# krea-ai/realtime-video

Measured on AMD Instinct MI355X. Metric: frames/sec at 832x480, 4-step 14B T2V (per-step DiT latency in config), higher is better.
Workload: dtype bf16

## Files before the change

### realtime_video_amd/csrc/gemm8.hip

```cpp
#include <atomic>
#include <mutex>
#include <type_traits>

#include "gemm_core.h"
#include "gemm_split.h"
#include "rtv_internal.h"

namespace rtv {

namespace g8 {
constexpr int BM = 256, BN = 256, BK = 64;
constexpr int HALF_BYTES = 128 * BK * 2;
constexpr int A_OFF = 0;
constexpr int W_OFF = 6 * HALF_BYTES;
constexpr int LDS_BYTES = 10 * HALF_BYTES;
constexpr int THREADS = 512;
__device__ __forceinline__ int swz(int row, int chunk) { return chunk ^ ((row >> 1) & 7); }
}

#ifdef RTV_GEMM_TIMELINE
__device__ unsigned long long* g_timeline = nullptr;
#endif

__device__ __forceinline__ void g8_tile_mn(int tiles_m, int tiles_n, int tile_id, int* mt, int* nt) {
#if RTV_G8_BALANCED_GROUPS
  const int ngrp = (tiles_m + 7) >> 3;
  const int gq = tiles_m / ngrp, gr = tiles_m - gq * ngrp;
  const int big = (gq + 1) * tiles_n;
  int first_m, gm, in_group;
  if (tile_id < gr * big) {
    const int group = tile_id / big;
    gm = gq + 1;
    first_m = group * gm;
    in_group = tile_id - group * big;
  } else {
    const int t = tile_id - gr * big, sm = gq * tiles_n, group = t / sm;
    gm = gq;
    first_m = gr * (gq + 1) + group * gq;
    in_group = t - group * sm;
  }
#else
  constexpr int GROUP_M = 8;
  const int per_group = GROUP_M * tiles_n;
  const int group = tile_id / per_group;
  const int first_m = group * GROUP_M;
  const int gm = min(tiles_m - first_m, GROUP_M);
  const int in_group = tile_id - group * per_group;
#endif
  *mt = first_m + in_group % gm;
  *nt = in_group / gm;
}

template <bool F16>
__device__ __forceinline__ void gemm8m_body(const GemmParams& p, const SplitArgs& sp, int m0, int n0, int tile_id, int seg, int unit,
                                            int kt_begin, int kt_end, bool is_split);

template <bool F16, bool SKIP_IDLE>
__global__ __launch_bounds__(g8::THREADS, 2) void gemm8_kernel(GemmParams p, SplitArgs sp) {
  using namespace g8;
  int bid0 = blockIdx.x;
  if (sp.pair_units) {
    if (bid0 < sp.pair_pad) {
      if (bid0 >= sp.pair_units) return;
#pragma unroll 1
      for (int j = 0; j < 2; ++j) {
        const int tn = 2 * bid0 + j;
        if (tn >= p.tiles_n) break;
        if (j) __syncthreads();
        gemm8m_body<F16>(p, sp, sp.pair_m0, tn * BN, 0, 0, -1, 0, p.K / BK, false);
      }
      return;
    }
    bid0 -= sp.pair_pad;
  }
  if (sp.half_tail) {
    const int nhu = 2 * sp.tail_tiles;
    if (sp.split_first) bid0 = bid0 < nhu ? sp.first_unit + bid0 : bid0 - nhu;
    if (bid0 >= sp.first_unit) {
      const int v = xcd_remap(bid0 - sp.first_unit, nhu);
      const int tile_id = sp.first_unit + (v >> 1);
      int mt, nt;
      g8_tile_mn(p.tiles_m, p.tiles_n, tile_id, &mt, &nt);
      const int m0h = mt * BM + (v & 1) * 128;
      if (m0h >= p.M) return;
      gemm8m_body<F16>(p, sp, m0h, nt * BN, tile_id, 0, -1, 0, p.K / BK, false);
      return;
    }
    sp.S = 1;
    sp.split_first = 0;
  }
#ifdef RTV_GEMM_TIMELINE
  const unsigned long long tl_t0 = __builtin_amdgcn_s_memrealtime();
  unsigned long long tl_t1 = 0;
#endif
  typedef TileCfg<256, 256, 64, 2, 4> Cfg;
  extern __shared__ __attribute__((aligned(16))) char smem[];

  const int tid = threadIdx.x;
  const int lane = tid & 63;
  const int wave = __builtin_amdgcn_readfirstlane(tid >> 6);
  const int wr = wave >> 2, wc = wave & 3;
  const int l31 = lane & 31, g = lane >> 5;

  const int nk_total = p.K / BK;
  int tile_id, seg, unit, kt_begin, kt_end;
  const bool is_split = split_unit_of_block(sp, bid0, nk_total, &tile_id, &unit, &seg, &kt_begin, &kt_end);
  int mt_, nt_;
  g8_tile_mn(p.tiles_m, p.tiles_n, tile_id, &mt_, &nt_);
  const int m0 = mt_ * BM;
  const int n0 = nt_ * BN;
  uint32_t src_off[4][2];
  {
    const int rsub = lane >> 3, cpos = lane & 7;
#pragma unroll
    for (int j = 0; j < 2; ++j) {
      const int row = j * 64 + wave * 8 + rsub;
      const int ch = swz(row, cpos) * 8;
#pragma unroll
      for (int h = 0; h < 2; ++h) {
        const int gm_row = min(m0 + h * 128 + row, p.M - 1);
        const int gn_row = min(n0 + h * 128 + row, p.N - 1);
        src_off[h][j] = ((uint32_t)gm_row * (uint32_t)p.lda + ch) * 2u;
        src_off[2 + h][j] = ((uint32_t)gn_row * (uint32_t)p.ldw + ch) * 2u;
      }
    }
  }
  __amdgpu_buffer_rsrc_t rsrcA = __builtin_amdgcn_make_buffer_rsrc((void*)p.A, 0, 0x7fffffff, 0x00020000);
  __amdgpu_buffer_rsrc_t rsrcW = __builtin_amdgcn_make_buffer_rsrc((void*)p.W, 0, 0x7fffffff, 0x00020000);
  auto stage_piece = [&](int kt, int a3, int h, int j, auto chk) {
    if (decltype(chk)::value && kt >= kt_end) return;
    const int slot = h < 2 ? A_OFF + (a3 * 2 + h) * HALF_BYTES : W_OFF + ((kt & 1) * 2 + (h - 2)) * HALF_BYTES;
    __builtin_amdgcn_raw_ptr_buffer_load_lds(h < 2 ? rsrcA : rsrcW, (RTV_LDS void*)(smem + slot + (j * 64 + wave * 8) * 128), 16,
                                             src_off[h][j], (unsigned)kt * (BK * 2), 0, 0);
  };

  const int b_row0 = (wc & 1) * 64;
  u32x4 af[2][4];
  u32x4 bfr[2][4];
  auto read_a = [&](int a3, int mq) {
    const char* s = smem + A_OFF + (a3 * 2 + wr) * HALF_BYTES;
#pragma unroll
    for (int mb = 0; mb < 2; ++mb) {
      const int row = mq * 64 + mb * 32 + l31;
#pragma unroll
      for (int ks = 0; ks < 4; ++ks) af[mb][ks] = *(const u32x4*)(s + row * 128 + (swz(row, ks * 2 + g) << 4));
    }
  };
  auto read_w = [&](int wb) {
    const char* s = smem + W_OFF + (wb * 2 + (wc >> 1)) * HALF_BYTES;
#pragma unroll
    for (int nq = 0; nq < 2; ++nq) {
      const int row = b_row0 + nq * 32 + l31;
#pragma unroll
      for (int ks = 0; ks < 4; ++ks) bfr[nq][ks] = *(const u32x4*)(s + row * 128 + (swz(row, ks * 2 + g) << 4));
    }
  };

  f32x16 acc[4][2];
#pragma unroll
  for (int mi = 0; mi < 4; ++mi)
#pragma unroll
    for (int ni = 0; ni < 2; ++ni)
#pragma unroll
      for (int r = 0; r < 16; ++r) acc[mi][ni][r] = 0.f;

#define G8_FENCE() __builtin_amdgcn_sched_barrier(0)
#define G8_BARRIER()                  \
  do {                                \
    G8_FENCE();                       \
    __builtin_amdgcn_s_barrier();     \
    G8_FENCE();                       \
  } while (0)
#define G8_LDS_DONE()                                   \
  do {                                                  \
    asm volatile("s_waitcnt lgkmcnt(0)" ::: "memory");  \
    G8_FENCE();                                         \
  } while (0)

  const bool idle_rows = SKIP_IDLE && m0 + wr * 128 >= p.M;
  auto mma_half = [&](int mq, int st_kt, int st_a3, int h0, auto chk) {
    __builtin_amdgcn_s_setprio(1);
    int n = 0;
#pragma unroll
    for (int ks = 0; ks < 4; ++ks)
#pragma unroll
      for (int nq = 0; nq < 2; ++nq)
#pragma unroll
        for (int mb = 0; mb < 2; ++mb) {
          acc[mq * 2 + mb][nq] = Mfma32<F16>::run(bfr[nq][ks], af[mb][ks], acc[mq * 2 + mb][nq]);
          ++n;
          if ((n & 3) == 2) {
            G8_FENCE();
            stage_piece(st_kt, st_a3, h0 + (n >> 3), (n >> 2) & 1, chk);
            G8_FENCE();
          }
        }
    __builtin_amdgcn_s_setprio(0);
  };

#pragma unroll
  for (int t = 0; t < 2; ++t)
#pragma unroll
    for (int hh = 0; hh < 4; ++hh) {
      const int h = (hh + 2) & 3;
      stage_piece(kt_begin + t, t, h, 0, std::true_type{});
      stage_piece(kt_begin + t, t, h, 1, std::true_type{});
    }
  if (kt_begin + 1 < kt_end) asm volatile("s_waitcnt vmcnt(8)" ::: "memory");
  else asm volatile("s_waitcnt vmcnt(0)" ::: "memory");
  G8_BARRIER();
  if (wr == 1) G8_BARRIER();

  int a3 = 0;
  auto k_tile = [&](const int kt, auto chk) {
    constexpr bool CHK = decltype(chk)::value;
    const int a3n = a3 == 0 ? 2 : a3 - 1;
    read_w(kt & 1);
    read_a(a3, 0);
    G8_LDS_DONE();
    G8_BARRIER();
    mma_half(0, kt + 2, a3n, 0, chk);
    G8_BARRIER();
    read_a(a3, 1);
    if (!CHK || kt + 2 < kt_end) asm volatile("s_waitcnt vmcnt(4)" ::: "memory");
    else asm volatile("s_waitcnt vmcnt(0)" ::: "memory");
    G8_LDS_DONE();
    G8_BARRIER();
    mma_half(1, kt + 2, a3n, 2, chk);
    G8_BARRIER();
    a3 = a3 == 2 ? 0 : a3 + 1;
  };
  auto idle_tile = [&](const int kt) {
    const int a3n = a3 == 0 ? 2 : a3 - 1;
    G8_BARRIER();
#pragma unroll
    for (int i = 0; i < 4; ++i) stage_piece(kt + 2, a3n, i >> 1, i & 1, std::true_type{});
    G8_BARRIER();
    if (kt + 2 < kt_end) asm volatile("s_waitcnt vmcnt(4)" ::: "memory");
    else asm volatile("s_waitcnt vmcnt(0)" ::: "memory");
    G8_BARRIER();
#pragma unroll
    for (int i = 0; i < 4; ++i) stage_piece(kt + 2, a3n, 2 + (i >> 1), i & 1, std::true_type{});
    G8_BARRIER();
    a3 = a3 == 2 ? 0 : a3 + 1;
  };
  int kt = kt_begin;
  if (idle_rows) {
    for (; kt < kt_end; ++kt) idle_tile(kt);
  } else {
    for (; kt + 2 < kt_end; ++kt) k_tile(kt, std::false_type{});
    for (; kt < kt_end; ++kt) k_tile(kt, std::true_type{});
  }
  if (wr == 0) G8_BARRIER();

#ifdef RTV_GEMM_TIMELINE
  tl_t1 = __builtin_amdgcn_s_memrealtime();
  bool reducer = true;
  if (is_split) reducer = split_k_reduce<4>(acc, sp, unit, seg, tile_id, smem, tid, wave, lane);
  if (!reducer) {
    if (g_timeline && tid == 0) {
      unsigned long long* t = g_timeline + (size_t)blockIdx.x * 4;
      t[0] = tl_t0;
      t[1] = tl_t1;
      t[2] = __builtin_amdgcn_s_memrealtime();
      t[3] = ((unsigned long long)(seg + 1) << 32) | (unsigned)tile_id;
    }
    return;
  }
#else
  if (is_split && !split_k_reduce<4>(acc, sp, unit, seg, tile_id, smem, tid, wave, lane)) return;
#endif

  const bool wide = !((p.ldc | (p.residual ? p.ldr : 0)) & 7) && !(((uintptr_t)p.C | (uintptr_t)p.residual) & 15);
  if (wide) {
    if (is_split) __syncthreads();
#ifdef RTV_GEMM_TIMELINE
    unsigned long long tl_mid = 0;
    store_tile_lds<F16, 4>(p, m0 + wr * 128, n0 + wc * 64, lane, smem + wave * (128 * 128), acc, &tl_mid);
    if (g_timeline && tid == 0) g_timeline[(size_t)blockIdx.x * 4 + 1] = tl_mid | (1ull << 63);
    tl_t1 = tl_t1 ? tl_t1 : 0;
    if (g_timeline && tid == 0) {
      unsigned long long* t = g_timeline + (size_t)blockIdx.x * 4;
      t[0] = tl_t0;
      t[2] = __builtin_amdgcn_s_memrealtime();
      t[3] = ((unsigned long long)(is_split ? seg + 1 : 0) << 32) | (unsigned)tile_id;
      g_timeline[(size_t)(gridDim.x + blockIdx.x) * 4] = tl_t1;
    }
    return;
#else
    store_tile_lds<F16, 4>(p, m0 + wr * 128, n0 + wc * 64, lane, smem + wave * (128 * 128), acc);
#endif
  } else {
    store_tile<F16, Cfg>(p, m0 + wr * 128, n0 + wc * 64, lane, acc);
  }
#ifdef RTV_GEMM_TIMELINE
  if (g_timeline && tid == 0) {
    unsigned long long* t = g_timeline + (size_t)blockIdx.x * 4;
    t[0] = tl_t0;
    t[1] = tl_t1;
    t[2] = __builtin_amdgcn_s_memrealtime();
    t[3] = ((unsigned long long)(is_split ? seg + 1 : 0) << 32) | (unsigned)tile_id | (is_split ? 0x80000000u : 0u);
  }
#endif
}

static std::atomic<bool> g_gemm8_skip_idle{true};
static std::atomic<bool> g_gemm8_half_tail{true};
static std::atomic<bool> g_gemm8_ragged_strips{true};
namespace g8m {
constexpr int BM = 128, BN = 256, BK = 64;
constexpr int HALF_BYTES = 128 * BK * 2;
constexpr int LDS_BYTES = 9 * HALF_BYTES;
}

template <bool F16>
__device__ __forceinline__ void gemm8m_body(const GemmParams& p, const SplitArgs& sp, int m0, int n0, int tile_id, int seg, int unit,
                                            int kt_begin, int kt_end, bool is_split) {
  using namespace g8m;
  extern __shared__ __attribute__((aligned(16))) char smem[];
  const int tid = threadIdx.x;
  const int lane = tid & 63;
  const int wave = __builtin_amdgcn_readfirstlane(tid >> 6);
  const int wr = wave >> 2, wc = wave & 3;
  const int l31 = lane & 31, g = lane >> 5;

  uint32_t src_off[3][2];
  {
    const int rsub = lane >> 3, cpos = lane & 7;
#pragma unroll
    for (int j = 0; j < 2; ++j) {
      const int row = j * 64 + wave * 8 + rsub;
      const int ch = g8::swz(row, cpos) * 8;
      src_off[0][j] = ((uint32_t)min(m0 + row, p.M - 1) * (uint32_t)p.lda + ch) * 2u;
      src_off[1][j] = ((uint32_t)min(n0 + row, p.N - 1) * (uint32_t)p.ldw + ch) * 2u;
      src_off[2][j] = ((uint32_t)min(n0 + 128 + row, p.N - 1) * (uint32_t)p.ldw + ch) * 2u;
    }
  }
  __amdgpu_buffer_rsrc_t rsrcA = __builtin_amdgcn_make_buffer_rsrc((void*)p.A, 0, 0x7fffffff, 0x00020000);
  __amdgpu_buffer_rsrc_t rsrcW = __builtin_amdgcn_make_buffer_rsrc((void*)p.W, 0, 0x7fffffff, 0x00020000);
  auto stage_piece = [&](int kt, int b3, int h, int j, auto chk) {
    if (decltype(chk)::value && kt >= kt_end) return;
    __builtin_amdgcn_raw_ptr_buffer_load_lds(h == 0 ? rsrcA : rsrcW,
                                             (RTV_LDS void*)(smem + (b3 * 3 + h) * HALF_BYTES + (j * 64 + wave * 8) * 128), 16,
                                             src_off[h][j], (unsigned)kt * (BK * 2), 0, 0);
  };

  u32x4 af[2][4], bfr[2][4];
  auto read_frags = [&](int b3) {
    const char* sa = smem + (b3 * 3) * HALF_BYTES;
    const char* sw = smem + (b3 * 3 + 1 + (wc >> 1)) * HALF_BYTES;
#pragma unroll
    for (int nq = 0; nq < 2; ++nq) {
      const int row = (wc & 1) * 64 + nq * 32 + l31;
#pragma unroll
      for (int ks = 0; ks < 4; ++ks) bfr[nq][ks] = *(const u32x4*)(sw + row * 128 + (g8::swz(row, ks * 2 + g) << 4));
    }
#pragma unroll
    for (int mb = 0; mb < 2; ++mb) {
      const int row = wr * 64 + mb * 32 + l31;
#pragma unroll
      for (int ks = 0; ks < 4; ++ks) af[mb][ks] = *(const u32x4*)(sa + row * 128 + (g8::swz(row, ks * 2 + g) << 4));
    }
  };

  f32x16 acc[2][2];
#pragma unroll
  for (int mi = 0; mi < 2; ++mi)
#pragma unroll
    for (int ni = 0; ni < 2; ++ni)
#pragma unroll
      for (int r = 0; r < 16; ++r) acc[mi][ni][r] = 0.f;

#pragma unroll
  for (int t = 0; t < 2; ++t)
#pragma unroll
    for (int h = 0; h < 3; ++h) {
      stage_piece(kt_begin + t, t, h, 0, std::true_type{});
      stage_piece(kt_begin + t, t, h, 1, std::true_type{});
    }
  if (wr == 1) {
#pragma unroll
    for (int h = 0; h < 3; ++h) {
      stage_piece(kt_begin + 2, 2, h, 0, std::true_type{});
      stage_piece(kt_begin + 2, 2, h, 1, std::true_type{});
    }
  }
  if (wr == 1) {
    if (kt_begin + 2 < kt_end) asm volatile("s_waitcnt vmcnt(6)" ::: "memory");
    else asm volatile("s_waitcnt vmcnt(0)" ::: "memory");
  } else {
    if (kt_begin + 1 < kt_end) asm volatile("s_waitcnt vmcnt(6)" ::: "memory");
    else asm volatile("s_waitcnt vmcnt(0)" ::: "memory");
  }
  G8_BARRIER();
  if (wr == 1) G8_BARRIER();

  int b3 = 0;
  auto k_tile = [&](const int kt, auto chk) {
    constexpr bool CHK = decltype(chk)::value;
    read_frags(b3);
    G8_LDS_DONE();
    G8_BARRIER();
    const int st_kt = kt + 2 + wr;
    const int st_b = wr ? b3 : (b3 == 0 ? 2 : b3 - 1);
    __builtin_amdgcn_s_setprio(1);
    int n = 0;
#pragma unroll
    for (int ks = 0; ks < 4; ++ks)
#pragma unroll
      for (int nq = 0; nq < 2; ++nq)
#pragma unroll
        for (int mb = 0; mb < 2; ++mb) {
          acc[mb][nq] = Mfma32<F16>::run(bfr[nq][ks], af[mb][ks], acc[mb][nq]);
          ++n;
          if (n == 2 || n == 4 || n == 7 || n == 10 || n == 12 || n == 15) {
            const int pc = n == 2 ? 0 : n == 4 ? 1 : n == 7 ? 2 : n == 10 ? 3 : n == 12 ? 4 : 5;
            G8_FENCE();
            stage_piece(st_kt, st_b, pc >> 1, pc & 1, chk);
            G8_FENCE();
          }
        }
    __builtin_amdgcn_s_setprio(0);
    G8_FENCE();
    if (!CHK || st_kt < kt_end) asm volatile("s_waitcnt vmcnt(6)" ::: "memory");
    else asm volatile("s_waitcnt vmcnt(0)" ::: "memory");
    G8_BARRIER();
    b3 = b3 == 2 ? 0 : b3 + 1;
  };
  int kt = kt_begin;
  for (; kt + 3 < kt_end; ++kt) k_tile(kt, std::false_type{});
  for (; kt < kt_end; ++kt) k_tile(kt, std::true_type{});
  if (wr == 0) G8_BARRIER();

  if (is_split && !split_k_reduce<2>(acc, sp, unit, seg, tile_id, smem, tid, wave, lane)) return;

  const bool wide = !((p.ldc | (p.residual ? p.ldr : 0)) & 7) && !(((uintptr_t)p.C | (uintptr_t)p.residual) & 15);
  if (wide) {
    if (is_split) __syncthreads();
    store_tile_lds<F16, 2>(p, m0 + wr * 64, n0 + wc * 64, lane, smem + wave * (64 * 128), acc);
  } else {
    typedef TileCfg<128, 256, 64, 2, 4> CfgM;
    store_tile<F16, CfgM>(p, m0 + wr * 64, n0 + wc * 64, lane, acc);
  }
}

template <bool F16>
__global__ __launch_bounds__(g8::THREADS, 2) void gemm8m_kernel(GemmParams p, SplitArgs sp) {
  using namespace g8m;
  const int nk_total = p.K / BK;
  int tile_id, seg, unit, kt_begin, kt_end;
  const bool is_split = split_unit_of_block(sp, blockIdx.x, nk_total, &tile_id, &unit, &seg, &kt_begin, &kt_end);
  constexpr int GROUP_M = 8;
  const int per_group = GROUP_M * p.tiles_n;
  const int group = tile_id / per_group;
  const int first_m = group * GROUP_M;
  const int gm = min(p.tiles_m - first_m, GROUP_M);
  const int in_group = tile_id - group * per_group;
  gemm8m_body<F16>(p, sp, (first_m + in_group % gm) * BM, (in_group / gm) * BN, tile_id, seg, unit, kt_begin, kt_end, is_split);
}

struct SplitWorkspace {
  int device;
  hipStream_t stream;
  bool any_stream;
  float* slabs;
  int* counters;
};
constexpr int MAX_WORKSPACES = 64;
constexpr int MAX_DEVICES = 64;
static SplitWorkspace g_ws[MAX_WORKSPACES];
static int g_num_ws = 0;
static std::mutex g_ws_mu;

static int attach_workspace(bool any_stream, hipStream_t stream, void* ptr, size_t bytes) {
  int dev = 0;
  if (hipGetDevice(&dev) != hipSuccess) return set_error(-1, "gemm_set_workspace: cannot query the device");
  std::lock_guard<std::mutex> lk(g_ws_mu);
  int slot = -1;
  for (int i = 0; i < g_num_ws; ++i)
    if (g_ws[i].device == dev && g_ws[i].any_stream == any_stream && (any_stream || g_ws[i].stream == stream)) slot = i;
  if (!ptr) {
    if (slot >= 0) g_ws[slot] = g_ws[--g_num_ws];
    return 0;
  }
  if (((uintptr_t)ptr) & 255) return set_error(-1, "gemm_set_workspace: pointer must be 256-byte aligned");
  if (bytes < rtv_gemm_workspace_bytes()) return set_error(-1, "gemm_set_workspace: too small (rtv_gemm_workspace_bytes)");
  if (slot < 0) {
    if (g_num_ws == MAX_WORKSPACES) return set_error(-1, "gemm_set_workspace: too many workspaces attached");
    slot = g_num_ws++;
  }
  SplitWorkspace w{dev, stream, any_stream, (float*)ptr, (int*)((char*)ptr + (size_t)SPLIT_MAX_UNITS * SPLIT_SLAB_FLOATS * 4)};
  if (hipMemset(w.counters, 0, (size_t)SPLIT_MAX_UNITS * sizeof(int)) != hipSuccess) {
    if (slot == g_num_ws - 1) --g_num_ws;
    return set_error(-1, "gemm_set_workspace: cannot zero the arrival counters");
  }
  g_ws[slot] = w;
  return 0;
}

}

using namespace rtv;

#ifdef RTV_GEMM_TIMELINE
extern "C" int rtv_gemm_debug_timeline(unsigned long long* buf) {
  return hipMemcpyToSymbol(HIP_SYMBOL(g_timeline), &buf, sizeof(buf)) == hipSuccess ? 0 : -1;
}
#endif

extern "C" int rtv_gemm_set_half_tail(int on) {
  rtv::g_gemm8_half_tail.store(on != 0, std::memory_order_relaxed);
  return 0;
}

extern "C" int rtv_gemm_set_ragged_strips(int on) {
  rtv::g_gemm8_ragged_strips.store(on != 0, std::memory_order_relaxed);
  return 0;
}

extern "C" int rtv_gemm_set_skip_idle(int on) {
  rtv::g_gemm8_skip_idle.store(on != 0, std::memory_order_relaxed);
  return 0;
}

extern "C" size_t rtv_gemm_workspace_bytes(void) {
  return (size_t)SPLIT_MAX_UNITS * SPLIT_SLAB_FLOATS * 4 + (size_t)SPLIT_MAX_UNITS * 4 + 256;
}

extern "C" int rtv_gemm_set_workspace(void* ptr, size_t bytes) { return attach_workspace(true, nullptr, ptr, bytes); }

extern "C" int rtv_gemm_set_stream_workspace(rtv_stream_t stream, void* ptr, size_t bytes) {
  return attach_workspace(false, (hipStream_t)stream, ptr, bytes);
}

namespace rtv {

int plan_split_k(int T, int nk, bool allow_split, SplitArgs* sp, int* grid, hipStream_t stream, bool allow_half, int extra_units) {
  int dev = 0;
  if (hipGetDevice(&dev) != hipSuccess || dev < 0 || dev >= MAX_DEVICES) return set_error(-1, "gemm: cannot query the device");
  float* slabs = nullptr;
  int* counters = nullptr;
  const int G = device_num_cus();
  if (G <= 0) return set_error(-1, "gemm: cannot query the device");
  {
    std::lock_guard<std::mutex> lk(g_ws_mu);
    for (int i = 0; i < g_num_ws && allow_split; ++i) {
      const SplitWorkspace& w = g_ws[i];
      if (w.device != dev) continue;
      if (!w.any_stream && w.stream == stream) {
        slabs = w.slabs;
        counters = w.counters;
        break;
      }
      if (w.any_stream && !slabs) {
        slabs = w.slabs;
        counters = w.counters;
      }
    }
  }
  *sp = SplitArgs{T, 1, nullptr, nullptr, 0, 0, 0, 0, 0, 0};
  *grid = T;
  const int R = (T + extra_units) % G <= T ? (T + extra_units) % G : 0;
  if (allow_half && g_gemm8_half_tail.load(std::memory_order_relaxed) && R > 0 && T > R && G / R == 2 && nk <= 128) {
    sp->first_unit = T - R;
    sp->tail_tiles = R;
    sp->half_tail = 1;
    *grid = (T - R) + 2 * R;
    return 0;
  }
  if (allow_split && slabs && R > 0) {
    int S = G / R;
    if (S > 8) S = 8;
    if (S > nk / 4) S = nk / 4;
    if (S >= 2 && (size_t)R * S <= (size_t)SPLIT_MAX_UNITS) {
      sp->first_unit = T - R;
      sp->S = S;
      sp->slabs = slabs;
      sp->counters = counters;
      sp->tail_tiles = R;
      sp->split_first = (R * S * 4 <= G) ? 1 : 0;
      *grid = (T - R) + R * S;
    }
  }
  return 0;
}

template <bool F16, bool SKIP_IDLE>
static int launch_gemm8_t(GemmParams p, bool allow_split, hipStream_t stream) {
  p.tiles_m = (p.M + g8::BM - 1) / g8::BM;
  p.tiles_n = (p.N + g8::BN - 1) / g8::BN;
  auto kern = gemm8_kernel<F16, SKIP_IDLE>;
  static LdsAttr lds_attr;
  if (int st = ensure_dynamic_lds((const void*)kern, g8::LDS_BYTES, &lds_attr, "gemm8")) return st;
  SplitArgs sp;
  int grid = 0;
// ... 59 lines not shown
```

### realtime_video_amd/csrc/gemm_core.h

```cpp
#pragma once
#include "rtv_common.h"

namespace rtv {

struct GemmParams {
  const uint16_t* A;
  const uint16_t* W;
  uint16_t* C;
  int lda, ldw, ldc;
  int M, N, K;
  const uint16_t* bias;
  int act;
  const uint16_t* gate;
  int gate_stride;
  int rows_per_frame;
  int row_offset;
  const uint16_t* residual;
  int ldr;
  int tiles_m, tiles_n;
};

template <bool F16>
struct Mfma32;
template <>
struct Mfma32<false> {
  static __device__ __forceinline__ f32x16 run(const u32x4& a, const u32x4& b, const f32x16& c) {
    return __builtin_amdgcn_mfma_f32_32x32x16_bf16(__builtin_bit_cast(bf16x8, a),
                                                   __builtin_bit_cast(bf16x8, b), c, 0, 0, 0);
  }
  static __device__ __forceinline__ float to_f32(uint16_t v) { return bf16_to_f32(v); }
  static __device__ __forceinline__ uint16_t from_f32(float v) { return f32_to_bf16(v); }
  static __device__ __forceinline__ float round(float v) { return round_bf16(v); }
  static __device__ __forceinline__ uint32_t pack2(float lo, float hi) { return pack_bf16x2(lo, hi); }
  static __device__ __forceinline__ float lo_f32(uint32_t u) { return __uint_as_float(u << 16); }
  static __device__ __forceinline__ float hi_f32(uint32_t u) { return __uint_as_float(u & 0xffff0000u); }
};
template <>
struct Mfma32<true> {
  static __device__ __forceinline__ f32x16 run(const u32x4& a, const u32x4& b, const f32x16& c) {
    return __builtin_amdgcn_mfma_f32_32x32x16_f16(__builtin_bit_cast(f16x8, a),
                                                  __builtin_bit_cast(f16x8, b), c, 0, 0, 0);
  }
  static __device__ __forceinline__ float to_f32(uint16_t v) { return f16_to_f32(v); }
  static __device__ __forceinline__ uint16_t from_f32(float v) { return f32_to_f16(v); }
  static __device__ __forceinline__ float round(float v) { return round_f16(v); }
  static __device__ __forceinline__ uint32_t pack2(float lo, float hi) { return pack_f16x2(lo, hi); }
  static __device__ __forceinline__ float lo_f32(uint32_t u) { return f16_to_f32((uint16_t)(u & 0xffff)); }
  static __device__ __forceinline__ float hi_f32(uint32_t u) { return f16_to_f32((uint16_t)(u >> 16)); }
};

template <int BM, int BN, int BK, int WM, int WN>
struct TileCfg {
  static constexpr int NW = WM * WN;
  static constexpr int NT = NW * 64;
  static constexpr int CH = BK / 8;
  static constexpr int RPI = 64 / CH;
  static constexpr int RPB = 16 / CH;
  static constexpr int A_INST = BM / RPI / NW;
  static constexpr int B_INST = BN / RPI / NW;
  static constexpr int A_BYTES = BM * BK * 2;
  static constexpr int B_BYTES = BN * BK * 2;
  static constexpr int STAGE_BYTES = A_BYTES + B_BYTES;
  static constexpr int TM = BM / WM / 32;
  static constexpr int TN = BN / WN / 32;
  static_assert(BM % (RPI * NW) == 0 && BN % (RPI * NW) == 0, "tile/wave mismatch");
  static_assert(BK % 16 == 0 && (CH == 4 || CH == 8), "BK must be 32 or 64");
  static __device__ __forceinline__ int swz(int row, int chunk) {
    return chunk ^ ((row / RPB) & (CH - 1));
  }
};

__device__ __forceinline__ void dma16(const void* gsrc, char* lds_wave_base) {
  __builtin_amdgcn_global_load_lds((const RTV_GLOBAL void*)gsrc, (RTV_LDS void*)lds_wave_base, 16, 0,
                                   0);
}

template <bool F16, typename Cfg, int BK>
__device__ __forceinline__ void mma_stage(const char* sA, const char* sB, int a_row0, int b_row0,
                                          int lane, f32x16 (&acc)[Cfg::TM][Cfg::TN]) {
  const int l31 = lane & 31, g = lane >> 5;
#pragma unroll
  for (int ks = 0; ks < BK / 16; ++ks) {
    u32x4 af[Cfg::TM], bf[Cfg::TN];
#pragma unroll
    for (int mi = 0; mi < Cfg::TM; ++mi) {
      int row = a_row0 + mi * 32 + l31;
      af[mi] = *(const u32x4*)(sA + row * (BK * 2) + Cfg::swz(row, ks * 2 + g) * 16);
    }
#pragma unroll
    for (int ni = 0; ni < Cfg::TN; ++ni) {
      int row = b_row0 + ni * 32 + l31;
      bf[ni] = *(const u32x4*)(sB + row * (BK * 2) + Cfg::swz(row, ks * 2 + g) * 16);
    }
#pragma unroll
    for (int mi = 0; mi < Cfg::TM; ++mi)
#pragma unroll
      for (int ni = 0; ni < Cfg::TN; ++ni)
        acc[mi][ni] = Mfma32<F16>::run(bf[ni], af[mi], acc[mi][ni]);
  }
}

template <bool F16>
__device__ __forceinline__ void epilogue_quad(const GemmParams& p, int m, int n, const float* v4) {
  typedef Mfma32<F16> T;
  float v[4] = {v4[0], v4[1], v4[2], v4[3]};
  if (p.bias) {
    u32x2 b = *(const u32x2*)(p.bias + n);
    v[0] += T::to_f32(b[0] & 0xffff);
    v[1] += T::to_f32(b[0] >> 16);
    v[2] += T::to_f32(b[1] & 0xffff);
    v[3] += T::to_f32(b[1] >> 16);
  }
#pragma unroll
  for (int i = 0; i < 4; ++i) v[i] = T::round(v[i]);
  if (p.act == 1) {
#pragma unroll
    for (int i = 0; i < 4; ++i) v[i] = T::round(gelu_tanh(v[i]));
  } else if (p.act == 2) {
#pragma unroll
    for (int i = 0; i < 4; ++i) v[i] = T::round(silu(v[i]));
  }
  if (p.gate) {
    const uint16_t* gp = p.gate + (size_t)((p.row_offset + m) / p.rows_per_frame) * p.gate_stride + n;
    u32x2 g = *(const u32x2*)gp;
    v[0] = T::round(v[0] * T::to_f32(g[0] & 0xffff));
    v[1] = T::round(v[1] * T::to_f32(g[0] >> 16));
    v[2] = T::round(v[2] * T::to_f32(g[1] & 0xffff));
    v[3] = T::round(v[3] * T::to_f32(g[1] >> 16));
  }
  if (p.residual) {
    u32x2 r = *(const u32x2*)(p.residual + (size_t)m * p.ldr + n);
    v[0] += T::to_f32(r[0] & 0xffff);
    v[1] += T::to_f32(r[0] >> 16);
    v[2] += T::to_f32(r[1] & 0xffff);
    v[3] += T::to_f32(r[1] >> 16);
  }
  u32x2 o;
  o[0] = (uint32_t)T::from_f32(v[0]) | ((uint32_t)T::from_f32(v[1]) << 16);
  o[1] = (uint32_t)T::from_f32(v[2]) | ((uint32_t)T::from_f32(v[3]) << 16);
  *(u32x2*)(p.C + (size_t)m * p.ldc + n) = o;
}

template <bool F16, typename Cfg>
__device__ __forceinline__ void store_tile(const GemmParams& p, int m_base, int n_base, int lane,
                                           f32x16 (&acc)[Cfg::TM][Cfg::TN]) {
  const int l31 = lane & 31, g = lane >> 5;
#pragma unroll
  for (int mi = 0; mi < Cfg::TM; ++mi) {
    int m = m_base + mi * 32 + l31;
    if (m >= p.M) continue;
#pragma unroll
    for (int ni = 0; ni < Cfg::TN; ++ni) {
#pragma unroll
      for (int rq = 0; rq < 4; ++rq) {
        int n = n_base + ni * 32 + rq * 8 + g * 4;
        if (n < p.N) {
          float v4[4] = {acc[mi][ni][rq * 4 + 0], acc[mi][ni][rq * 4 + 1], acc[mi][ni][rq * 4 + 2],
                         acc[mi][ni][rq * 4 + 3]};
          epilogue_quad<F16>(p, m, n, v4);
        }
      }
    }
  }
}

template <bool F16, int TM, int ACT, bool GATE>
__device__ __forceinline__ void store_tile_lds_impl(const GemmParams& p, int m_base, int n_base, int lane, char* img,
                                                    f32x16 (&acc)[TM][2], unsigned long long* mid_stamp) {
  typedef Mfma32<F16> T;
  const int l31 = lane & 31, g = lane >> 5;
  int ncol[8];
  u32x2 bq[8];
#pragma unroll
  for (int s8 = 0; s8 < 8; ++s8) {
    ncol[s8] = min(n_base + (s8 >> 2) * 32 + (s8 & 3) * 8 + g * 4, p.N - 4);
    bq[s8] = p.bias ? *(const u32x2*)(p.bias + ncol[s8]) : u32x2{0u, 0u};
  }
#pragma unroll
  for (int mi = 0; mi < TM; ++mi) {
    const int row = mi * 32 + l31;
    u32x2 gq[8];
    if (GATE) {
      const uint16_t* gp = p.gate + (size_t)((p.row_offset + min(m_base + row, p.M - 1)) / p.rows_per_frame) * p.gate_stride;
#pragma unroll
      for (int s8 = 0; s8 < 8; ++s8) gq[s8] = *(const u32x2*)(gp + ncol[s8]);
    }
#pragma unroll
    for (int ni = 0; ni < 2; ++ni)
#pragma unroll
      for (int rq = 0; rq < 4; ++rq) {
        const int s8 = ni * 4 + rq;
        float v[4] = {acc[mi][ni][rq * 4 + 0], acc[mi][ni][rq * 4 + 1], acc[mi][ni][rq * 4 + 2], acc[mi][ni][rq * 4 + 3]};
        v[0] += T::lo_f32(bq[s8][0]);
        v[1] += T::hi_f32(bq[s8][0]);
        v[2] += T::lo_f32(bq[s8][1]);
        v[3] += T::hi_f32(bq[s8][1]);
        if (ACT == 1) {
#pragma unroll
          for (int i = 0; i < 4; ++i) v[i] = gelu_tanh(T::round(v[i]));
        } else if (ACT == 2) {
#pragma unroll
          for (int i = 0; i < 4; ++i) v[i] = silu(T::round(v[i]));
        }
        if (GATE) {
          v[0] = T::round(v[0]) * T::lo_f32(gq[s8][0]);
          v[1] = T::round(v[1]) * T::hi_f32(gq[s8][0]);
          v[2] = T::round(v[2]) * T::lo_f32(gq[s8][1]);
          v[3] = T::round(v[3]) * T::hi_f32(gq[s8][1]);
        }
        u32x2 o;
        o[0] = T::pack2(v[0], v[1]);
        o[1] = T::pack2(v[2], v[3]);
        const int chunk = s8 ^ (row & 7);
        const int half = g ^ ((row >> 3) & 1);
        *(u32x2*)(img + row * 128 + chunk * 16 + half * 8) = o;
      }
  }
  asm volatile("s_waitcnt lgkmcnt(0)" ::: "memory");
  __builtin_amdgcn_sched_barrier(0);
  if (mid_stamp) *mid_stamp = __builtin_amdgcn_s_memrealtime();
  const int rsub = lane >> 3, c = lane & 7;
  const int n = n_base + c * 8;
  const bool n_ok = n < p.N;
  constexpr int PASSES = TM * 4;
  u32x4 res[PASSES];
  if (p.residual) {
#pragma unroll
    for (int ps = 0; ps < PASSES; ++ps) {
      const int m = min(m_base + ps * 8 + rsub, p.M - 1);
      res[ps] = *(const u32x4*)(p.residual + (size_t)m * p.ldr + min(n, p.N - 8));
    }
  }
#pragma unroll
  for (int ps = 0; ps < PASSES; ++ps) {
    const int row = ps * 8 + rsub;
    const int m = m_base + row;
    u32x4 t = *(const u32x4*)(img + row * 128 + ((c ^ (row & 7)) << 4));
    if ((row >> 3) & 1) t = u32x4{t[2], t[3], t[0], t[1]};
    if (p.residual) {
#pragma unroll
      for (int i = 0; i < 4; ++i)
        t[i] = T::pack2(T::lo_f32(t[i]) + T::lo_f32(res[ps][i]), T::hi_f32(t[i]) + T::hi_f32(res[ps][i]));
    }
    if (m < p.M && n_ok) *(u32x4*)(p.C + (size_t)m * p.ldc + n) = t;
  }
}

template <bool F16, int TM>
__device__ __forceinline__ void store_tile_lds(const GemmParams& p, int m_base, int n_base, int lane, char* img,
                                               f32x16 (&acc)[TM][2], unsigned long long* mid_stamp = nullptr) {
  if (p.gate) {
    if (p.act == 0) store_tile_lds_impl<F16, TM, 0, true>(p, m_base, n_base, lane, img, acc, mid_stamp);
    else if (p.act == 1) store_tile_lds_impl<F16, TM, 1, true>(p, m_base, n_base, lane, img, acc, mid_stamp);
    else store_tile_lds_impl<F16, TM, 2, true>(p, m_base, n_base, lane, img, acc, mid_stamp);
  } else {
    if (p.act == 0) store_tile_lds_impl<F16, TM, 0, false>(p, m_base, n_base, lane, img, acc, mid_stamp);
    else if (p.act == 1) store_tile_lds_impl<F16, TM, 1, false>(p, m_base, n_base, lane, img, acc, mid_stamp);
    else store_tile_lds_impl<F16, TM, 2, false>(p, m_base, n_base, lane, img, acc, mid_stamp);
  }
}

}
```

### realtime_video_amd/csrc/gemm_split.h

```cpp
#pragma once
#include "rtv_common.h"

namespace rtv {

constexpr int SPLIT_SLAB_FLOATS = 256 * 256;
constexpr int SPLIT_MAX_UNITS = 256;

struct SplitArgs {
  int first_unit;
  int S;
  float* slabs;
  int* counters;
  int tail_tiles;
  int split_first;
  int half_tail;
  int pair_units;
  int pair_pad;
  int pair_m0;
};

int plan_split_k(int T, int nk, bool allow_split, SplitArgs* sp, int* grid, hipStream_t stream, bool allow_half = false,
                 int extra_units = 0);

__device__ __forceinline__ bool split_unit_of_block(const SplitArgs& sp, int bid, int nk_total, int* tile_id, int* unit,
                                                    int* seg, int* kt_begin, int* kt_end) {
  *seg = 0;
  *unit = -1;
  if (sp.split_first) {
    const int nsu = sp.tail_tiles * sp.S;
    bid = bid < nsu ? sp.first_unit + bid : bid - nsu;
  }
  if (bid < sp.first_unit) {
    *tile_id = xcd_remap(bid, sp.first_unit);
  } else {
    const int v = xcd_remap(bid - sp.first_unit, sp.tail_tiles * sp.S);
    *seg = v / sp.tail_tiles;
    const int tl = v - *seg * sp.tail_tiles;
    *tile_id = sp.first_unit + tl;
    *unit = tl * sp.S + *seg;
  }
  const bool is_split = *unit >= 0 && sp.S > 1;
  *kt_begin = is_split ? (int)((long)nk_total * *seg / sp.S) : 0;
  *kt_end = is_split ? (int)((long)nk_total * (*seg + 1) / sp.S) : nk_total;
  return is_split;
}

template <int TM>
__device__ __forceinline__ bool split_k_reduce(f32x16 (&acc)[TM][2], const SplitArgs& sp, int unit, int seg, int tile_id,
                                               char* smem, int tid, int wave, int lane) {
  constexpr int NB = TM * 2;
  __amdgpu_buffer_rsrc_t slab =
      __builtin_amdgcn_make_buffer_rsrc((void*)(sp.slabs + (size_t)unit * SPLIT_SLAB_FLOATS), 0, SPLIT_SLAB_FLOATS * 4, 0x00020000);
#pragma unroll
  for (int blk = 0; blk < NB; ++blk)
#pragma unroll
    for (int q = 0; q < 4; ++q) {
      const f32x16& a = acc[blk >> 1][blk & 1];
      const f32x4 v = {a[4 * q], a[4 * q + 1], a[4 * q + 2], a[4 * q + 3]};
      __builtin_amdgcn_raw_buffer_store_b128(__builtin_bit_cast(u32x4, v), slab, (((wave * NB + blk) * 4 + q) * 64 + lane) * 16, 0,
                                              16);
    }
  asm volatile("s_waitcnt vmcnt(0)" ::: "memory");
  __syncthreads();
  int* flag = (int*)smem;
  if (tid == 0)
    *flag = __hip_atomic_fetch_add(sp.counters + (tile_id - sp.first_unit), 1, __ATOMIC_RELAXED, __HIP_MEMORY_SCOPE_AGENT);
  __syncthreads();
  const int ticket = *flag;
  if (ticket != sp.S - 1) return false;
  if (tid == 0) {
    __builtin_amdgcn_fence(__ATOMIC_ACQUIRE, "agent");
    __hip_atomic_store(sp.counters + (tile_id - sp.first_unit), 0, __ATOMIC_RELAXED, __HIP_MEMORY_SCOPE_AGENT);
  }
  __syncthreads();
  const int unit0 = unit - seg;
  if (sp.S > 2) {
#pragma unroll
    for (int blk = 0; blk < NB; ++blk)
#pragma unroll
      for (int r = 0; r < 16; ++r) acc[blk >> 1][blk & 1][r] = 0.f;
  }
  for (int s = 0; s < sp.S; ++s) {
    if (s == seg && sp.S == 2) continue;
    const float4* other = (const float4*)(sp.slabs + (size_t)(unit0 + s) * SPLIT_SLAB_FLOATS);
#pragma unroll
    for (int blk = 0; blk < NB; ++blk)
#pragma unroll
      for (int q = 0; q < 4; ++q) {
        const float4 v = other[((wave * NB + blk) * 4 + q) * 64 + lane];
        f32x16& a = acc[blk >> 1][blk & 1];
        a[4 * q] += v.x;
        a[4 * q + 1] += v.y;
        a[4 * q + 2] += v.z;
        a[4 * q + 3] += v.w;
      }
  }
  return true;
}

}
```

Before: 18.56.

## Switch gemm8 kernels from 32x32x16 to 16x16x32 MFMA with matching epilogues

Replaces the 32x32 MFMA instruction in both gemm8 kernels with the 16x16x32 variant, reorganizing fragment loads, accumulator layout, the interleaving of global-to-LDS staging with MFMAs, the split-K reduction and the tile store epilogues to fit the new 16x16 accumulator shape. It is enabled by default through a compile macro. The intent is higher MFMA throughput or better latency behavior on MI355X for these shapes. It adds more, smaller instructions and LDS reads, and changes register pressure and how staging overlaps with compute.

After: 18.85 (median of 6 runs). +1.6%, better.

```diff
diff --git a/realtime_video_amd/csrc/gemm8.hip b/realtime_video_amd/csrc/gemm8.hip
--- a/realtime_video_amd/csrc/gemm8.hip
+++ b/realtime_video_amd/csrc/gemm8.hip
@@ -5,6 +5,10 @@
 #include "gemm_core.h"
 #include "gemm_split.h"
 #include "rtv_internal.h"
+
+#ifndef RTV_G8_MFMA16
+#define RTV_G8_MFMA16 1
+#endif
 
 namespace rtv {
 
@@ -91,16 +95,17 @@
   }
 #ifdef RTV_GEMM_TIMELINE
   const unsigned long long tl_t0 = __builtin_amdgcn_s_memrealtime();
+  const unsigned long long tl_c0 = __builtin_amdgcn_s_memtime();
   unsigned long long tl_t1 = 0;
 #endif
-  typedef TileCfg<256, 256, 64, 2, 4> Cfg;
+  [[maybe_unused]] typedef TileCfg<256, 256, 64, 2, 4> Cfg;
   extern __shared__ __attribute__((aligned(16))) char smem[];
 
   const int tid = threadIdx.x;
   const int lane = tid & 63;
   const int wave = __builtin_amdgcn_readfirstlane(tid >> 6);
   const int wr = wave >> 2, wc = wave & 3;
-  const int l31 = lane & 31, g = lane >> 5;
+  [[maybe_unused]] const int l31 = lane & 31, g = lane >> 5;
 
   const int nk_total = p.K / BK;
   int tile_id, seg, unit, kt_begin, kt_end;
@@ -135,6 +140,37 @@
   };
 
   const int b_row0 = (wc & 1) * 64;
+#if RTV_G8_MFMA16
+  const int l15 = lane & 15, q4 = lane >> 4;
+  u32x4 af[4][2];
+  u32x4 bfr[4][2];
+  auto read_a = [&](int a3, int mq) {
+    const char* s = smem + A_OFF + (a3 * 2 + wr) * HALF_BYTES;
+#pragma unroll
+    for (int mb = 0; mb < 4; ++mb) {
+      const int row = mq * 64 + mb * 16 + l15;
+#pragma unroll
+      for (int ks = 0; ks < 2; ++ks) af[mb][ks] = *(const u32x4*)(s + row * 128 + (swz(row, ks * 4 + q4) << 4));
+    }
+  };
+  auto read_w = [&](int wb) {
+    const char* s = smem + W_OFF + (wb * 2 + (wc >> 1)) * HALF_BYTES;
+#pragma unroll
+    for (int nb = 0; nb < 4; ++nb) {
+      const int row = b_row0 + nb * 16 + l15;
+#pragma unroll
+      for (int ks = 0; ks < 2; ++ks) bfr[nb][ks] = *(const u32x4*)(s + row * 128 + (swz(row, ks * 4 + q4) << 4));
+    }
+  };
+
+  f32x4 acc[8][4];
+#pragma unroll
+  for (int mi = 0; mi < 8; ++mi)
+#pragma unroll
+    for (int ni = 0; ni < 4; ++ni)
+#pragma unroll
+      for (int r = 0; r < 4; ++r) acc[mi][ni][r] = 0.f;
+#else
   u32x4 af[2][4];
   u32x4 bfr[2][4];
   auto read_a = [&](int a3, int mq) {
@@ -163,8 +199,16 @@
     for (int ni = 0; ni < 2; ++ni)
 #pragma unroll
       for (int r = 0; r < 16; ++r) acc[mi][ni][r] = 0.f;
+#endif
 
 #define G8_FENCE() __builtin_amdgcn_sched_barrier(0)
+#if RTV_G8_MFMA16
+#define G8_STORE_LDS(...) store_tile_lds16<F16>(__VA_ARGS__)
+#define G8_STORE_DIRECT(CFG, ...) store_tile16<F16>(__VA_ARGS__)
+#else
+#define G8_STORE_LDS(...) store_tile_lds<F16>(__VA_ARGS__)
+#define G8_STORE_DIRECT(CFG, ...) store_tile<F16, CFG>(__VA_ARGS__)
+#endif
 #define G8_BARRIER()                  \
   do {                                \
     G8_FENCE();                       \
@@ -181,6 +225,22 @@
   auto mma_half = [&](int mq, int st_kt, int st_a3, int h0, auto chk) {
     __builtin_amdgcn_s_setprio(1);
     int n = 0;
+#if RTV_G8_MFMA16
+#pragma unroll
+    for (int ks = 0; ks < 2; ++ks)
+#pragma unroll
+      for (int nb = 0; nb < 4; ++nb)
+#pragma unroll
+        for (int mb = 0; mb < 4; ++mb) {
+          acc[mq * 4 + mb][nb] = Mfma16<F16>::run(bfr[nb][ks], af[mb][ks], acc[mq * 4 + mb][nb]);
+          ++n;
+          if ((n & 7) == 4) {
+            G8_FENCE();
+            stage_piece(st_kt, st_a3, h0 + (n >> 4), (n >> 3) & 1, chk);
+            G8_FENCE();
+          }
+        }
+#else
 #pragma unroll
     for (int ks = 0; ks < 4; ++ks)
 #pragma unroll
@@ -195,6 +255,7 @@
             G8_FENCE();
           }
         }
+#endif
     __builtin_amdgcn_s_setprio(0);
   };
 
@@ -255,8 +316,9 @@
 
 #ifdef RTV_GEMM_TIMELINE
   tl_t1 = __builtin_amdgcn_s_memrealtime();
+  const unsigned long long tl_c1 = __builtin_amdgcn_s_memtime();
   bool reducer = true;
-  if (is_split) reducer = split_k_reduce<4>(acc, sp, unit, seg, tile_id, smem, tid, wave, lane);
+  if (is_split) reducer = split_k_reduce(acc, sp, unit, seg, tile_id, smem, tid, wave, lane);
   if (!reducer) {
     if (g_timeline && tid == 0) {
       unsigned long long* t = g_timeline + (size_t)blockIdx.x * 4;
@@ -268,7 +330,7 @@
     return;
   }
 #else
-  if (is_split && !split_k_reduce<4>(acc, sp, unit, seg, tile_id, smem, tid, wave, lane)) return;
+  if (is_split && !split_k_reduce(acc, sp, unit, seg, tile_id, smem, tid, wave, lane)) return;
 #endif
 
   const bool wide = !((p.ldc | (p.residual ? p.ldr : 0)) & 7) && !(((uintptr_t)p.C | (uintptr_t)p.residual) & 15);
@@ -276,7 +338,7 @@
     if (is_split) __syncthreads();
 #ifdef RTV_GEMM_TIMELINE
     unsigned long long tl_mid = 0;
-    store_tile_lds<F16, 4>(p, m0 + wr * 128, n0 + wc * 64, lane, smem + wave * (128 * 128), acc, &tl_mid);
+    G8_STORE_LDS(p, m0 + wr * 128, n0 + wc * 64, lane, smem + wave * (128 * 128), acc, &tl_mid);
     if (g_timeline && tid == 0) g_timeline[(size_t)blockIdx.x * 4 + 1] = tl_mid | (1ull << 63);
     tl_t1 = tl_t1 ? tl_t1 : 0;
     if (g_timeline && tid == 0) {
@@ -285,13 +347,14 @@
       t[2] = __builtin_amdgcn_s_memrealtime();
       t[3] = ((unsigned long long)(is_split ? seg + 1 : 0) << 32) | (unsigned)tile_id;
       g_timeline[(size_t)(gridDim.x + blockIdx.x) * 4] = tl_t1;
+      g_timeline[(size_t)(gridDim.x + blockIdx.x) * 4 + 1] = tl_c1 - tl_c0;
     }
     return;
 #else
-    store_tile_lds<F16, 4>(p, m0 + wr * 128, n0 + wc * 64, lane, smem + wave * (128 * 128), acc);
+    G8_STORE_LDS(p, m0 + wr * 128, n0 + wc * 64, lane, smem + wave * (128 * 128), acc, nullptr);
 #endif
   } else {
-    store_tile<F16, Cfg>(p, m0 + wr * 128, n0 + wc * 64, lane, acc);
+    G8_STORE_DIRECT(Cfg, p, m0 + wr * 128, n0 + wc * 64, lane, acc);
   }
 #ifdef RTV_GEMM_TIMELINE
   if (g_timeline && tid == 0) {
@@ -322,7 +385,7 @@
   const int lane = tid & 63;
   const int wave = __builtin_amdgcn_readfirstlane(tid >> 6);
   const int wr = wave >> 2, wc = wave & 3;
-  const int l31 = lane & 31, g = lane >> 5;
+  [[maybe_unused]] const int l31 = lane & 31, g = lane >> 5;
 
   uint32_t src_off[3][2];
   {
@@ -345,6 +408,34 @@
                                              src_off[h][j], (unsigned)kt * (BK * 2), 0, 0);
   };
 
+#if RTV_G8_MFMA16
+  const int l15 = lane & 15, q4 = lane >> 4;
+  u32x4 af[4][2], bfr[4][2];
+  auto read_frags = [&](int b3) {
+    const char* sa = smem + (b3 * 3) * HALF_BYTES;
+    const char* sw = smem + (b3 * 3 + 1 + (wc >> 1)) * HALF_BYTES;
+#pragma unroll
+    for (int nb = 0; nb < 4; ++nb) {
+      const int row = (wc & 1) * 64 + nb * 16 + l15;
+#pragma unroll
+      for (int ks = 0; ks < 2; ++ks) bfr[nb][ks] = *(const u32x4*)(sw + row * 128 + (g8::swz(row, ks * 4 + q4) << 4));
+    }
+#pragma unroll
+    for (int mb = 0; mb < 4; ++mb) {
+      const int row = wr * 64 + mb * 16 + l15;
+#pragma unroll
+      for (int ks = 0; ks < 2; ++ks) af[mb][ks] = *(const u32x4*)(sa + row * 128 + (g8::swz(row, ks * 4 + q4) << 4));
+    }
+  };
+
+  f32x4 acc[4][4];
+#pragma unroll
+  for (int mi = 0; mi < 4; ++mi)
+#pragma unroll
+    for (int ni = 0; ni < 4; ++ni)
+#pragma unroll
+      for (int r = 0; r < 4; ++r) acc[mi][ni][r] = 0.f;
+#else
   u32x4 af[2][4], bfr[2][4];
   auto read_frags = [&](int b3) {
     const char* sa = smem + (b3 * 3) * HALF_BYTES;
@@ -370,6 +461,7 @@
     for (int ni = 0; ni < 2; ++ni)
 #pragma unroll
       for (int r = 0; r < 16; ++r) acc[mi][ni][r] = 0.f;
+#endif
 
 #pragma unroll
   for (int t = 0; t < 2; ++t)
@@ -405,6 +497,23 @@
     const int st_b = wr ? b3 : (b3 == 0 ? 2 : b3 - 1);
     __builtin_amdgcn_s_setprio(1);
     int n = 0;
+#if RTV_G8_MFMA16
+#pragma unroll
+    for (int ks = 0; ks < 2; ++ks)
+#pragma unroll
+      for (int nb = 0; nb < 4; ++nb)
+#pragma unroll
+        for (int mb = 0; mb < 4; ++mb) {
+          acc[mb][nb] = Mfma16<F16>::run(bfr[nb][ks], af[mb][ks], acc[mb][nb]);
+          ++n;
+          if (n == 4 || n == 8 || n == 14 || n == 20 || n == 24 || n == 30) {
+            const int pc = n == 4 ? 0 : n == 8 ? 1 : n == 14 ? 2 : n == 20 ? 3 : n == 24 ? 4 : 5;
+            G8_FENCE();
+            stage_piece(st_kt, st_b, pc >> 1, pc & 1, chk);
+            G8_FENCE();
+          }
+        }
+#else
 #pragma unroll
     for (int ks = 0; ks < 4; ++ks)
 #pragma unroll
@@ -420,6 +529,7 @@
             G8_FENCE();
           }
         }
+#endif
     __builtin_amdgcn_s_setprio(0);
     G8_FENCE();
     if (!CHK || st_kt < kt_end) asm volatile("s_waitcnt vmcnt(6)" ::: "memory");
@@ -432,15 +542,15 @@
   for (; kt < kt_end; ++kt) k_tile(kt, std::true_type{});
   if (wr == 0) G8_BARRIER();
 
-  if (is_split && !split_k_reduce<2>(acc, sp, unit, seg, tile_id, smem, tid, wave, lane)) return;
+  if (is_split && !split_k_reduce(acc, sp, unit, seg, tile_id, smem, tid, wave, lane)) return;
 
   const bool wide = !((p.ldc | (p.residual ? p.ldr : 0)) & 7) && !(((uintptr_t)p.C | (uintptr_t)p.residual) & 15);
   if (wide) {
     if (is_split) __syncthreads();
-    store_tile_lds<F16, 2>(p, m0 + wr * 64, n0 + wc * 64, lane, smem + wave * (64 * 128), acc);
+    G8_STORE_LDS(p, m0 + wr * 64, n0 + wc * 64, lane, smem + wave * (64 * 128), acc, nullptr);
   } else {
-    typedef TileCfg<128, 256, 64, 2, 4> CfgM;
-    store_tile<F16, CfgM>(p, m0 + wr * 64, n0 + wc * 64, lane, acc);
+    [[maybe_unused]] typedef TileCfg<128, 256, 64, 2, 4> CfgM;
+    G8_STORE_DIRECT(CfgM, p, m0 + wr * 64, n0 + wc * 64, lane, acc);
   }
 }
 
diff --git a/realtime_video_amd/csrc/gemm_core.h b/realtime_video_amd/csrc/gemm_core.h
--- a/realtime_video_amd/csrc/gemm_core.h
+++ b/realtime_video_amd/csrc/gemm_core.h
@@ -47,6 +47,14 @@
   static __device__ __forceinline__ uint32_t pack2(float lo, float hi) { return pack_f16x2(lo, hi); }
   static __device__ __forceinline__ float lo_f32(uint32_t u) { return f16_to_f32((uint16_t)(u & 0xffff)); }
   static __device__ __forceinline__ float hi_f32(uint32_t u) { return f16_to_f32((uint16_t)(u >> 16)); }
+};
+
+template <bool F16>
+struct Mfma16 : Mfma32<F16> {
+  static __device__ __forceinline__ f32x4 run(const u32x4& a, const u32x4& b, const f32x4& c) {
+    if constexpr (F16) return __builtin_amdgcn_mfma_f32_16x16x32_f16(__builtin_bit_cast(f16x8, a), __builtin_bit_cast(f16x8, b), c, 0, 0, 0);
+    else return __builtin_amdgcn_mfma_f32_16x16x32_bf16(__builtin_bit_cast(bf16x8, a), __builtin_bit_cast(bf16x8, b), c, 0, 0, 0);
+  }
 };
 
 template <int BM, int BN, int BK, int WM, int WN>
@@ -260,4 +268,113 @@
   }
 }
 
-}
+template <bool F16, int TMB>
+__device__ __forceinline__ void store_tile16(const GemmParams& p, int m_base, int n_base, int lane, f32x4 (&acc)[TMB][4]) {
+  const int l15 = lane & 15, q = lane >> 4;
+#pragma unroll
+  for (int mb = 0; mb < TMB; ++mb) {
+    const int m = m_base + mb * 16 + l15;
+    if (m >= p.M) continue;
+#pragma unroll
+    for (int nb = 0; nb < 4; ++nb) {
+      const int n = n_base + nb * 16 + q * 4;
+      if (n < p.N) {
+        float v4[4] = {acc[mb][nb][0], acc[mb][nb][1], acc[mb][nb][2], acc[mb][nb][3]};
+        epilogue_quad<F16>(p, m, n, v4);
+      }
+    }
+  }
+}
+
+template <bool F16, int TMB, int ACT, bool GATE>
+__device__ __forceinline__ void store_tile_lds16_impl(const GemmParams& p, int m_base, int n_base, int lane, char* img,
+                                                      f32x4 (&acc)[TMB][4], unsigned long long* mid_stamp) {
+  typedef Mfma32<F16> T;
+  const int l15 = lane & 15, q = lane >> 4;
+  int ncol[4];
+  u32x2 bq[4];
+#pragma unroll
+  for (int nb = 0; nb < 4; ++nb) {
+    ncol[nb] = min(n_base + nb * 16 + q * 4, p.N - 4);
+    bq[nb] = p.bias ? *(const u32x2*)(p.bias + ncol[nb]) : u32x2{0u, 0u};
+  }
+#pragma unroll
+  for (int mb = 0; mb < TMB; ++mb) {
+    const int row = mb * 16 + l15;
+    u32x2 gq[4];
+    if (GATE) {
+      const uint16_t* gp = p.gate + (size_t)((p.row_offset + min(m_base + row, p.M - 1)) / p.rows_per_frame) * p.gate_stride;
+#pragma unroll
+      for (int nb = 0; nb < 4; ++nb) gq[nb] = *(const u32x2*)(gp + ncol[nb]);
+    }
+#pragma unroll
+    for (int nb = 0; nb < 4; ++nb) {
+      float v[4] = {acc[mb][nb][0], acc[mb][nb][1], acc[mb][nb][2], acc[mb][nb][3]};
+      v[0] += T::lo_f32(bq[nb][0]);
+      v[1] += T::hi_f32(bq[nb][0]);
+      v[2] += T::lo_f32(bq[nb][1]);
+      v[3] += T::hi_f32(bq[nb][1]);
+      if (ACT == 1) {
+#pragma unroll
+        for (int i = 0; i < 4; ++i) v[i] = gelu_tanh(T::round(v[i]));
+      } else if (ACT == 2) {
+#pragma unroll
+        for (int i = 0; i < 4; ++i) v[i] = silu(T::round(v[i]));
+      }
+      if (GATE) {
+        v[0] = T::round(v[0]) * T::lo_f32(gq[nb][0]);
+        v[1] = T::round(v[1]) * T::hi_f32(gq[nb][0]);
+        v[2] = T::round(v[2]) * T::lo_f32(gq[nb][1]);
+        v[3] = T::round(v[3]) * T::hi_f32(gq[nb][1]);
+      }
+      u32x2 o;
+      o[0] = T::pack2(v[0], v[1]);
+      o[1] = T::pack2(v[2], v[3]);
+      *(u32x2*)(img + row * 128 + (((nb * 4 + q) ^ l15) << 3)) = o;
+    }
+  }
+  asm volatile("s_waitcnt lgkmcnt(0)" ::: "memory");
+  __builtin_amdgcn_sched_barrier(0);
+  if (mid_stamp) *mid_stamp = __builtin_amdgcn_s_memrealtime();
+  const int rsub = lane >> 3, c = lane & 7;
+  const int n = n_base + c * 8;
+  const bool n_ok = n < p.N;
+  constexpr int PASSES = TMB * 2;
+  u32x4 res[PASSES];
+  if (p.residual) {
+#pragma unroll
+    for (int ps = 0; ps < PASSES; ++ps) {
+      const int m = min(m_base + ps * 8 + rsub, p.M - 1);
+      res[ps] = *(const u32x4*)(p.residual + (size_t)m * p.ldr + min(n, p.N - 8));
+    }
+  }
+#pragma unroll
+  for (int ps = 0; ps < PASSES; ++ps) {
+    const int row = ps * 8 + rsub;
+    const int m = m_base + row;
+    u32x4 t = *(const u32x4*)(img + row * 128 + ((c ^ ((row >> 1) & 7)) << 4));
+    if (row & 1) t = u32x4{t[2], t[3], t[0], t[1]};
+    if (p.residual) {
+#pragma unroll
+      for (int i = 0; i < 4; ++i)
+        t[i] = T::pack2(T::lo_f32(t[i]) + T::lo_f32(res[ps][i]), T::hi_f32(t[i]) + T::hi_f32(res[ps][i]));
+    }
+    if (m < p.M && n_ok) *(u32x4*)(p.C + (size_t)m * p.ldc + n) = t;
+  }
+}
+
+template <bool F16, int TMB>
+__device__ __forceinline__ void store_tile_lds16(const GemmParams& p, int m_base, int n_base, int lane, char* img,
+                                                 f32x4 (&acc)[TMB][4], unsigned long long* mid_stamp = nullptr) {
+  if (p.gate) {
+    if (p.act == 0) store_tile_lds16_impl<F16, TMB, 0, true>(p, m_base, n_base, lane, img, acc, mid_stamp);
+    else if (p.act == 1) store_tile_lds16_impl<F16, TMB, 1, true>(p, m_base, n_base, lane, img, acc, mid_stamp);
+    else store_tile_lds16_impl<F16, TMB, 2, true>(p, m_base, n_base, lane, img, acc, mid_stamp);
+  } else {
+    if (p.act == 0) store_tile_lds16_impl<F16, TMB, 0, false>(p, m_base, n_base, lane, img, acc, mid_stamp);
+    else if (p.act == 1) store_tile_lds16_impl<F16, TMB, 1, false>(p, m_base, n_base, lane, img, acc, mid_stamp);
+    else store_tile_lds16_impl<F16, TMB, 2, false>(p, m_base, n_base, lane, img, acc, mid_stamp);
+  }
+}
+
+}
diff --git a/realtime_video_amd/csrc/gemm_split.h b/realtime_video_amd/csrc/gemm_split.h
--- a/realtime_video_amd/csrc/gemm_split.h
+++ b/realtime_video_amd/csrc/gemm_split.h
@@ -45,21 +45,16 @@
   return is_split;
 }
 
-template <int TM>
-__device__ __forceinline__ bool split_k_reduce(f32x16 (&acc)[TM][2], const SplitArgs& sp, int unit, int seg, int tile_id,
-                                               char* smem, int tid, int wave, int lane) {
-  constexpr int NB = TM * 2;
+template <int NQ, class Get, class Set>
+__device__ __forceinline__ bool split_k_reduce_quads(Get get, Set set, const SplitArgs& sp, int unit, int seg, int tile_id,
+                                                     char* smem, int tid, int wave, int lane) {
   __amdgpu_buffer_rsrc_t slab =
       __builtin_amdgcn_make_buffer_rsrc((void*)(sp.slabs + (size_t)unit * SPLIT_SLAB_FLOATS), 0, SPLIT_SLAB_FLOATS * 4, 0x00020000);
 #pragma unroll
-  for (int blk = 0; blk < NB; ++blk)
-#pragma unroll
-    for (int q = 0; q < 4; ++q) {
-      const f32x16& a = acc[blk >> 1][blk & 1];
-      const f32x4 v = {a[4 * q], a[4 * q + 1], a[4 * q + 2], a[4 * q + 3]};
-      __builtin_amdgcn_raw_buffer_store_b128(__builtin_bit_cast(u32x4, v), slab, (((wave * NB + blk) * 4 + q) * 64 + lane) * 16, 0,
-                                              16);
-    }
+  for (int qi = 0; qi < NQ; ++qi) {
+    const f32x4 v = get(qi);
+    __builtin_amdgcn_raw_buffer_store_b128(__builtin_bit_cast(u32x4, v), slab, ((wave * NQ + qi) * 64 + lane) * 16, 0,  16);
+  }
   asm volatile("s_waitcnt vmcnt(0)" ::: "memory");
   __syncthreads();
   int* flag = (int*)smem;
@@ -76,26 +71,48 @@
   const int unit0 = unit - seg;
   if (sp.S > 2) {
 #pragma unroll
-    for (int blk = 0; blk < NB; ++blk)
-#pragma unroll
-      for (int r = 0; r < 16; ++r) acc[blk >> 1][blk & 1][r] = 0.f;
+    for (int qi = 0; qi < NQ; ++qi) set(qi, f32x4{0.f, 0.f, 0.f, 0.f});
   }
   for (int s = 0; s < sp.S; ++s) {
     if (s == seg && sp.S == 2) continue;
     const float4* other = (const float4*)(sp.slabs + (size_t)(unit0 + s) * SPLIT_SLAB_FLOATS);
 #pragma unroll
-    for (int blk = 0; blk < NB; ++blk)
-#pragma unroll
-      for (int q = 0; q < 4; ++q) {
-        const float4 v = other[((wave * NB + blk) * 4 + q) * 64 + lane];
-        f32x16& a = acc[blk >> 1][blk & 1];
-        a[4 * q] += v.x;
-        a[4 * q + 1] += v.y;
-        a[4 * q + 2] += v.z;
-        a[4 * q + 3] += v.w;
-      }
+    for (int qi = 0; qi < NQ; ++qi) {
+      const float4 v = other[(wave * NQ + qi) * 64 + lane];
+      f32x4 a = get(qi);
+      a[0] += v.x;
+      a[1] += v.y;
+      a[2] += v.z;
+      a[3] += v.w;
+      set(qi, a);
+    }
   }
   return true;
 }
 
+template <int TM>
+__device__ __forceinline__ bool split_k_reduce(f32x16 (&acc)[TM][2], const SplitArgs& sp, int unit, int seg, int tile_id,
+                                               char* smem, int tid, int wave, int lane) {
+  return split_k_reduce_quads<TM * 8>(
+      [&](int qi) __attribute__((always_inline)) {
+        const f32x16& a = acc[qi >> 3][(qi >> 2) & 1];
+        const int q = qi & 3;
+        return f32x4{a[4 * q], a[4 * q + 1], a[4 * q + 2], a[4 * q + 3]};
+      },
+      [&](int qi, f32x4 v) __attribute__((always_inline)) {
+        f32x16& a = acc[qi >> 3][(qi >> 2) & 1];
+        const int q = qi & 3;
+        a[4 * q] = v[0], a[4 * q + 1] = v[1], a[4 * q + 2] = v[2], a[4 * q + 3] = v[3];
+      },
+      sp, unit, seg, tile_id, smem, tid, wave, lane);
 }
+
+template <int TMB>
+__device__ __forceinline__ bool split_k_reduce(f32x4 (&acc)[TMB][4], const SplitArgs& sp, int unit, int seg, int tile_id,
+                                               char* smem, int tid, int wave, int lane) {
+  return split_k_reduce_quads<TMB * 4>([&](int qi) __attribute__((always_inline)) { return acc[qi >> 2][qi & 3]; },
+                                       [&](int qi, f32x4 v) __attribute__((always_inline)) { acc[qi >> 2][qi & 3] = v; }, sp, unit, seg,
+                                       tile_id, smem, tid, wave, lane);
+}
+
+}
```
